# rvp-group/mad-icp

Hardware: NVIDIA H100
Metric: scans/sec (130k-pt scan vs 16-keyframe model) (higher is better)
Workload: dtype f64

## Files before the change

mad_icp_b200/csrc/capi.cu:

```cuda
#include <cooperative_groups.h>
#include <cuda_runtime.h>

#include <algorithm>
#include <cmath>
#include <cstdio>
#include <cstdlib>
#include <cstring>
#include <new>
#include <stdexcept>
#include <string>
#include <vector>

#include "../../include/madicp_b200_debug.h"
#include "ctx.hpp"
#include "device_kernels.cuh"

namespace madicp {

static thread_local std::string g_error;
void set_error(const std::string& msg) { g_error = msg; }

}

using namespace madicp;

ModelView madicp_make_view(const madicp_ctx* c) {
  ModelView v;
  v.recs = c->d_pool_recs;
  v.quad = c->d_quad;
  v.ww = c->d_pool_ww;
  v.K = 0;
  for (int s = 0; s < c->max_keyframes; ++s)
    if (c->slots[s].n_nodes > 0) {
      v.broot[v.K] = int(size_t(s) * c->pool_cap);
      v.qroot[v.K] = int(size_t(s) * c->quad_cap);
      ++v.K;
    }
  for (int i = v.K; i < kMaxSlots; ++i) v.broot[i] = v.qroot[i] = 0;
  return v;
}
static ModelView make_view(const madicp_ctx* c) { return madicp_make_view(c); }

static int blocks_for(int64_t n) { return int((n + kStepBlock - 1) / kStepBlock); }

static int prepare_slot(madicp_ctx* c, int s) {
  const int n = c->slots[s].n_nodes;
  const size_t off = size_t(s) * c->pool_cap;
  k_prepare_slot<<<blocks_for(n), kStepBlock, 0, c->stream>>>(
      c->d_pool_recs + off, n, int(off), c->P.min_ball, c->d_pool_lvl + size_t(s) * (kMaxLevels + 1),
      c->slots[s].n_levels, c->d_pool_child0 + off, c->d_pool_rec_of + off, c->d_quad + size_t(s) * c->quad_cap,
      c->d_pool_ww + off);
  c->launches++;
  CK(cudaGetLastError());
  return MADICP_OK;
}

static int build_slot(madicp_ctx* c, int s, const madtree_rec_t* src, const double* X_dev) {
  const int n = c->slots[s].n_nodes;
  const size_t off = size_t(s) * c->pool_cap;
  const int* lvl = c->d_pool_lvl + size_t(s) * (kMaxLevels + 1);
  const int nl = c->slots[s].n_levels;
  madtree_rec_t* dst = c->d_pool_recs + off;
  k_slot_ingest<<<blocks_for(n), kStepBlock, 0, c->stream>>>(src ? src : dst, dst, n, X_dev, lvl, nl, c->d_pool_child0 + off);
  k_quad_scan<<<1, 1024, 0, c->stream>>>(c->d_pool_child0 + off, n);
  k_quad_place<<<blocks_for(n), kStepBlock, 0, c->stream>>>(dst, n, lvl, nl, c->d_pool_child0 + off, c->d_pool_rec_of + off);
  c->launches += 3;
  CK(cudaGetLastError());
  return prepare_slot(c, s);
}

static int ensure_pool(madicp_ctx* c, size_t need) {
  if (need <= c->pool_cap) return MADICP_OK;
  CK(cudaStreamSynchronize(c->stream));
  size_t cap = size_t(1) << 16;
  while (cap + 40 < need || cap + 40 <= c->pool_cap) cap <<= 1;
  cap += 40;
  if (cap * size_t(c->max_keyframes) > size_t(0x3fffffff)) {
    set_error("keyframe pool would exceed 2^30 nodes");
    return MADICP_ERR_NOMEM;
  }
  madtree_rec_t* recs = nullptr;
  int *child0 = nullptr, *rec_of = nullptr;
  QuadRec* quad = nullptr;
  double* ww = nullptr;
  const size_t total = cap * size_t(c->max_keyframes);
  CK(cudaMalloc(&recs, total * sizeof(madtree_rec_t)));
  CK(cudaMalloc(&child0, total * sizeof(int)));
  CK(cudaMalloc(&rec_of, total * sizeof(int)));
  CK(cudaMalloc(&quad, 2 * total * sizeof(QuadRec)));
  CK(cudaMalloc(&ww, total * sizeof(double)));
  for (int s = 0; s < c->max_keyframes; ++s)
    if (c->slots[s].n_nodes > 0)
      CK(cudaMemcpyAsync(recs + size_t(s) * cap, c->d_pool_recs + size_t(s) * c->pool_cap,
                         size_t(c->slots[s].n_nodes) * sizeof(madtree_rec_t), cudaMemcpyDeviceToDevice, c->stream));
  CK(cudaStreamSynchronize(c->stream));
  cudaFree(c->d_pool_recs);
  cudaFree(c->d_pool_child0);
  cudaFree(c->d_pool_rec_of);
  cudaFree(c->d_quad);
  cudaFree(c->d_pool_ww);
  c->d_pool_ww = ww;
  c->d_pool_recs = recs;
  c->d_pool_child0 = child0;
  c->d_pool_rec_of = rec_of;
  c->d_quad = quad;
  c->quad_cap = 2 * cap;
  c->pool_cap = cap;
  for (int s = 0; s < c->max_keyframes; ++s)
    if (c->slots[s].n_nodes > 0) {
      int rc = build_slot(c, s, nullptr, nullptr);
      if (rc) return rc;
    }
  return MADICP_OK;
}

static int stage_pose(madicp_ctx* c, const double X[12], const double** X_dev) {
  const int r = int(c->xform_seq % madicp_ctx::kXformRing);
  if (c->xform_seq >= madicp_ctx::kXformRing) CK(cudaEventSynchronize(c->xform_done[r]));
  memcpy(c->h_xform + size_t(r) * 12, X, 12 * sizeof(double));
  CK(cudaMemcpyAsync(c->d_xform + size_t(r) * 12, c->h_xform + size_t(r) * 12, 12 * sizeof(double), cudaMemcpyHostToDevice,
                     c->stream));
  CK(cudaEventRecord(c->xform_done[r], c->stream));
  *X_dev = c->d_xform + size_t(r) * 12;
  c->xform_seq++;
  return MADICP_OK;
}

static int slot_rank(const madicp_ctx* c, int slot) {
  int k = 0;
  for (int s = 0; s < slot; ++s) k += (c->slots[s].n_nodes > 0);
  return k;
}

static int ensure_items(madicp_ctx* c, size_t items) {
  if (items <= c->cap_items) return MADICP_OK;
  CK(cudaStreamSynchronize(c->stream));
  if (c->d_hit) cudaFree(c->d_hit);
  if (c->d_ord) cudaFree(c->d_ord);
  c->d_hit = c->d_ord = nullptr;
  c->cap_items = 0;
  CK(cudaMalloc(&c->d_hit, items * sizeof(int)));
  CK(cudaMalloc(&c->d_ord, items * sizeof(int)));
  c->cap_items = items;
  return MADICP_OK;
}

struct GnShape {
  int threads, ctas;
  const void* fn;
  size_t smem;
};
template <int THREADS, int CTAS>
static GnShape gn_shape() {
  return GnShape{THREADS, CTAS, reinterpret_cast<const void*>(k_gn_loop<THREADS, CTAS>), gn_dynamic_smem<THREADS>()};
// ... 88 lines not shown
  c->max_keyframes = max_keyframes;
  c->sm_count = prop.multiProcessorCount;
  c->slots.resize(max_keyframes);
  {
    int lo_pri = 0, hi_pri = 0;
    CK(cudaDeviceGetStreamPriorityRange(&lo_pri, &hi_pri));
    CK(cudaStreamCreateWithPriority(&c->own_stream, cudaStreamNonBlocking, hi_pri));
  }
  c->stream = c->own_stream;
  CK(cudaMalloc(&c->d_state, sizeof(GnState)));
  CK(cudaMemset(c->d_state, 0, sizeof(GnState)));
  CK(cudaMalloc(&c->d_X, sizeof(double) * 64));
  CK(cudaMalloc(&c->d_comm, sizeof(CommBlock)));
  CK(cudaMemset(c->d_comm, 0, sizeof(CommBlock)));
  CK(cudaEventCreateWithFlags(&c->tree_free_ev, cudaEventDisableTiming));
  CK(cudaMalloc(&c->d_pool_lvl, size_t(max_keyframes) * (kMaxLevels + 1) * sizeof(int)));
  CK(cudaMalloc(&c->d_xform, size_t(madicp_ctx::kXformRing) * 12 * sizeof(double)));
  CK(cudaMallocHost(&c->h_xform, size_t(madicp_ctx::kXformRing) * 12 * sizeof(double)));
  CK(cudaMallocHost(&c->h_lvl, size_t(madicp_ctx::kXformRing) * (kMaxLevels + 1) * sizeof(int)));
  for (int i = 0; i < madicp_ctx::kXformRing; ++i) CK(cudaEventCreateWithFlags(&c->xform_done[i], cudaEventDisableTiming));
  CK(cudaMallocHost(&c->h_pinned, sizeof(double) * 64));
  CK(cudaMallocHost(&c->h_state, sizeof(GnState)));
  CK(cudaMallocHost(&c->h_matched, kMatchedCap));
  if (const char* e = getenv("MADICP_NO_MEMO")) c->memo_mode = (atoi(e) == 0) ? 2 : 0;
  int threads = 1024, ctas = 1;
  if (const char* e = getenv("MADICP_GN_SHAPE"))
    if (sscanf(e, "%d,%d", &threads, &ctas) == 2) c->gn_auto = false;
  int rc = configure_gn(c, threads, ctas);
  if (rc) return rc;
  c->cap_partial = size_t(c->sm_count) * 8 * kAcc;
  CK(cudaMalloc(&c->d_partial, c->cap_partial * sizeof(double)));
  CK(cudaMalloc(&c->d_tiles, c->cap_partial * sizeof(LLCell)));
  CK(cudaMemset(c->d_tiles, 0, c->cap_partial * sizeof(LLCell)));
  c->peer_comm[0] = c->d_comm;
  *out = c;
  return MADICP_OK;
  MADICP_CATCH("madicp_create")
}

void madicp_destroy(madicp_ctx_t* c) {
  if (!c) return;
  cudaSetDevice(c->device);
  cudaStreamSynchronize(c->stream);
  for (int r = 0; r < c->world; ++r)
    if (c->world > 1 && r != c->rank && c->peer_comm[r]) cudaIpcCloseMemHandle(c->peer_comm[r]);
  madicp_gpu_build_release(c);
  for (madtree_gpu* t : c->tree_cache) delete t;
  for (void* slab : c->tree_slabs) cudaFree(slab);
  cudaFree(c->d_pool_recs);
  cudaFree(c->d_pool_child0);
  cudaFree(c->d_pool_rec_of);
  cudaFree(c->d_pool_lvl);
  cudaFree(c->d_quad);
  cudaFree(c->d_pool_ww);
  cudaFree(c->d_xform);
  cudaFree(c->d_dbg_cta);
  cudaFree(c->d_moving);
  cudaFree(c->d_mov4);
  cudaFree(c->d_step_matched);
  cudaFree(c->d_hit);
  cudaFree(c->d_ord);
  cudaFree(c->d_cloud_q);
  cudaFree(c->d_cloud_o);
  cudaFree(c->d_partial);
  cudaFree(c->d_tiles);
  cudaFree(c->d_memo_leaf);
  cudaFree(c->d_memo_margin);
  cudaFree(c->d_memo_ckpt);
  cudaFree(c->d_memo_ckpt_up);
  cudaFree(c->d_state);
  cudaFree(c->d_X);
  cudaFree(c->d_comm);
  cudaFree(c->d_dbg);
  cudaFreeHost(c->h_xform);
  cudaFreeHost(c->h_lvl);
  cudaFreeHost(c->h_pinned);
  cudaFreeHost(c->h_state);
  for (int i = 0; i < madicp_ctx::kXformRing; ++i)
    if (c->xform_done[i]) cudaEventDestroy(c->xform_done[i]);
  cudaFreeHost(c->h_matched);
  if (c->tree_free_ev) cudaEventDestroy(c->tree_free_ev);
  cudaStreamDestroy(c->own_stream);
  delete c;
}

int madicp_set_params(madicp_ctx_t* c, double min_ball, double rho_ker, double b_ratio) {
  if (!c || !(min_ball > 0) || rho_ker < 0) {
    set_error("madicp_set_params: bad arguments");
    return MADICP_ERR_INVALID;
  }
  const bool reweigh = (min_ball != c->P.min_ball);
  c->P.min_ball = min_ball;
  c->P.rho_ker_sqrt = sqrt(rho_ker);
  c->P.b_ratio = b_ratio;
  c->mov4_stale = true;
  if (reweigh) {
    CK(cudaSetDevice(c->device));
    for (int s = 0; s < c->max_keyframes; ++s)
      if (c->slots[s].n_nodes > 0) {
        int rc = prepare_slot(c, s);
        if (rc) return rc;
      }
  }
  return MADICP_OK;
}

int madicp_set_stream(madicp_ctx_t* c, void* s) {
  if (!c) return MADICP_ERR_INVALID;
  c->stream = s ? static_cast<cudaStream_t>(s) : c->own_stream;
  return MADICP_OK;
}
void* madicp_get_stream(const madicp_ctx_t* c) { return c ? static_cast<void*>(c->stream) : nullptr; }
int madicp_synchronize(madicp_ctx_t* c) {
  if (!c) return MADICP_ERR_INVALID;
  CK(cudaSetDevice(c->device));
  CK(cudaStreamSynchronize(c->stream));
  return MADICP_OK;
}

static int level_table(const madtree_rec_t* recs, int n_nodes, int n_leaves, std::vector<int>& lvl) {
  lvl.clear();
  lvl.push_back(0);
// ... 441 lines not shown
  CK(cudaMemcpyAsync(c->h_pinned, c->d_X, 12 * sizeof(double), cudaMemcpyDeviceToHost, c->stream));
  CK(cudaStreamSynchronize(c->stream));
  memcpy(X, c->h_pinned, 12 * sizeof(double));
  return MADICP_OK;
}

static int register_enqueue(madicp_ctx* c, int iters, const double X0[12], int clear_from) {
  int rc = check_ready(c, "madicp_register");
  if (rc) return rc;
  if (!X0 || iters < 1 || iters > MADICP_MAX_ITERS) {
    set_error("madicp_register: bad arguments (1 <= iters <= 64 per launch)");
    return MADICP_ERR_INVALID;
  }
  CK(cudaSetDevice(c->device));
  rc = prepare_moving(c);
  if (rc) return rc;
  rc = pick_shape(c, int64_t(madicp_num_keyframes(c)) * c->L);
  if (rc) return rc;
  GnArgs A;
  A.model = make_view(c);
  A.P = c->P;
  A.peers.rank = c->rank;
  A.peers.world = c->world;
  A.peers.epoch_base = c->epoch;
  const int mb = int(c->call_seq & 1u);
  for (int r = 0; r < kMaxPeers; ++r) {
    A.peers.box[r] = (r < c->world) ? &c->peer_comm[r]->box : nullptr;
    A.peer_matched[r] = (r < c->world) ? c->peer_comm[r]->matched[mb] : nullptr;
  }
  A.moving = c->d_mov4;
  A.L = c->L;
  A.iters = iters;
  A.clear_from = clear_from;
  A.matched = c->d_comm->matched[mb];
  size_t map_bytes = 0;
  {
    const size_t per_cta = size_t(madicp_num_keyframes(c)) * (size_t(c->L) / size_t(c->gn_grid) + 8) * 4 + 128;
    auto bucket = [](size_t bytes) {
      const size_t kb[] = {8, 16, 32, 64, 100, 132, 164, 196, 228};
      for (size_t b : kb)
        if (bytes + 1024 <= b * 1024) return b;
      return size_t(1 << 20);
    };
    const size_t ctas = size_t(c->gn_grid / c->sm_count);
    if (per_cta <= kGnMapMaxBytes && c->L < (1 << 26) && bucket((c->gn_smem + per_cta) * ctas) == bucket(c->gn_smem * ctas))
      map_bytes = per_cta;
  }
  A.map_in_smem = map_bytes ? 1 : 0;
  {
    const size_t stride = ((size_t(c->max_keyframes) * (c->cap_moving / size_t(c->gn_grid) + 8)) + 31) & ~size_t(31);
    const size_t need = stride * size_t(c->gn_grid);
    if (need > c->cap_memo) {
      CK(cudaStreamSynchronize(c->stream));
      cudaFree(c->d_memo_leaf);
      cudaFree(c->d_memo_margin);
      cudaFree(c->d_memo_ckpt);
      cudaFree(c->d_memo_ckpt_up);
      c->d_memo_leaf = nullptr;
      c->d_memo_margin = nullptr;
      c->d_memo_ckpt = nullptr;
      c->d_memo_ckpt_up = nullptr;
      c->cap_memo = 0;
      const size_t cap = need + need / 4;
      CK(cudaMalloc(&c->d_memo_leaf, cap * sizeof(int)));
      CK(cudaMalloc(&c->d_memo_margin, cap * sizeof(float)));
      CK(cudaMalloc(&c->d_memo_ckpt, cap * sizeof(unsigned)));
      CK(cudaMalloc(&c->d_memo_ckpt_up, cap * sizeof(float)));
      c->cap_memo = cap;
    }
    A.memo_leaf = c->d_memo_leaf;
    A.memo_margin = c->d_memo_margin;
    A.memo_ckpt = c->d_memo_ckpt;
    A.memo_ckpt_up = c->d_memo_ckpt_up;
    A.item_stride = int(stride);
    A.memo_mode = c->memo_mode;
    A.walk_buf = mb;
  }
  A.st = c->d_state;
  A.dbg = c->d_dbg;
  A.dbg_cta = c->d_dbg ? c->d_dbg_cta : nullptr;
  c->epoch += uint32_t(iters);
  A.pose_epoch = c->pose_epoch;
  c->pose_epoch += uint32_t(iters);
  memcpy(A.X0, X0, 12 * sizeof(double));
  A.tiles = c->d_tiles;
  A.zero_next = c->d_comm->matched[mb ^ 1];
  A.zero_bytes = int((std::min(kMatchedCap, c->cap_moving) + 15) & ~size_t(15));
  void* args[] = {&A};
  CK(cudaLaunchCooperativeKernel(c->gn_kernel, dim3(c->gn_grid), dim3(c->gn_threads), args, c->gn_smem + map_bytes, c->stream));
  c->launches++;
  c->last_iters = iters;
  c->call_seq++;
  return MADICP_OK;
}

int madicp_register_async(madicp_ctx_t* c, int iters, const double X0[12]) {
  return register_enqueue(c, iters, X0, iters - 1);
}
int madicp_register_partial_async(madicp_ctx_t* c, int iters, const double X0[12]) {
  return register_enqueue(c, iters, X0, 0);
}

int madicp_register_fetch_weight(madicp_ctx_t* c, double X[12], double H[36], double b[6], uint8_t* matched, int* n_matched,
                                 double* weight) {
  if (!c || c->last_iters < 1) {
    set_error("madicp_register_fetch: nothing was enqueued");
    return MADICP_ERR_STATE;
  }
  CK(cudaSetDevice(c->device));
  CK(cudaMemcpyAsync(c->h_state, c->d_state, offsetof(GnState, X_trace), cudaMemcpyDeviceToHost, c->stream));
  if (matched)
    CK(cudaMemcpyAsync(c->h_matched, c->d_comm->matched[(c->call_seq - 1u) & 1u], size_t(c->L), cudaMemcpyDeviceToHost,
                       c->stream));
  CK(cudaStreamSynchronize(c->stream));
  if (c->h_state->error) {
    set_error("madicp_register: a peer GPU never delivered its H/b tile (rank down, or no matching registration enqueued there)");
    CK(cudaMemsetAsync(&c->d_state->error, 0, sizeof(int), c->stream));
    return MADICP_ERR_COMM;
  }
  if (X) memcpy(X, c->h_state->X_out, 12 * sizeof(double));
  if (H) memcpy(H, c->h_state->H, 36 * sizeof(double));
  if (b) memcpy(b, c->h_state->b, 6 * sizeof(double));
  if (matched) memcpy(matched, c->h_matched, size_t(c->L));
  if (n_matched) *n_matched = c->h_state->n_matched;
  if (weight) *weight = c->h_state->weight;
  return MADICP_OK;
// ... 256 lines not shown
```

mad_icp_b200/csrc/ctx.hpp:

```cpp
#pragma once
#include <cuda_runtime.h>

#include <atomic>
#include <mutex>
#include <new>
#include <stdexcept>
#include <string>
#include <vector>

#include "kernels.cuh"

namespace madicp {
void set_error(const std::string& msg);

constexpr int kMaxLevels = 4096;
struct Slot {
  int n_nodes = 0, n_leaves = 0, n_levels = 0;
};
constexpr size_t kMatchedCap = size_t(1) << 20;

struct CommBlock {
  Mailbox box;
  unsigned char matched[2][kMatchedCap];
};
}

struct madicp_ctx;

struct madtree_gpu {
  madicp_ctx* ctx = nullptr;
  madtree_rec_t* recs = nullptr;
  int* lvl = nullptr;
  int* leaf_of = nullptr;
  size_t cap_nodes = 0;
  void* block = nullptr;
  int n_nodes = 0, n_leaves = 0, n_levels = 0;
  std::vector<int> h_lvl;
  double* full = nullptr;
  int64_t n_points = 0;
  uint64_t build_seq = 0;
};

struct madicp_ctx {
  int device = 0;
  int max_keyframes = 0;
  cudaStream_t own_stream = nullptr, stream = nullptr;
  int sm_count = 0;
  std::vector<madicp::Slot> slots;
  size_t pool_cap = 0;
  madtree_rec_t* d_pool_recs = nullptr;
  int* d_pool_child0 = nullptr;
  int* d_pool_rec_of = nullptr;
  int* d_pool_lvl = nullptr;
  size_t quad_cap = 0;
  madicp::QuadRec* d_quad = nullptr;
  double* d_pool_ww = nullptr;
  static constexpr int kXformRing = 64;
  double* d_xform = nullptr;
  double* h_xform = nullptr;
  int* h_lvl = nullptr;
  cudaEvent_t xform_done[kXformRing] = {};
  uint32_t xform_seq = 0;
  std::vector<madtree_gpu*> tree_cache;
  std::vector<void*> tree_slabs;
  cudaEvent_t tree_free_ev = nullptr;
  std::mutex tree_mu;
  void* build_state = nullptr;
  long long* d_dbg_cta = nullptr;
  madicp::IcpParams P{0.2, 0.31622776601683794, 0.02};
  double* d_moving = nullptr;
  madicp::Moving4* d_mov4 = nullptr;
  bool mov4_stale = true;
  unsigned char* d_step_matched = nullptr;
  int L = 0;
  size_t cap_moving = 0;
  uint32_t call_seq = 0;
  int* d_hit = nullptr;
  int* d_ord = nullptr;
  size_t cap_items = 0;
  double* d_cloud_q = nullptr;
  int* d_cloud_o = nullptr;
  size_t cap_cloud = 0;
  double* d_partial = nullptr;
  madicp::LLCell* d_tiles = nullptr;
  size_t cap_partial = 0;
  int* d_memo_leaf = nullptr;
  float* d_memo_margin = nullptr;
  unsigned* d_memo_ckpt = nullptr;
  float* d_memo_ckpt_up = nullptr;
  size_t cap_memo = 0;
  int memo_mode = 2;
  madicp::GnState* d_state = nullptr;
  double* d_X = nullptr;
  madicp::CommBlock* d_comm = nullptr;
  double* h_pinned = nullptr;
  madicp::GnState* h_state = nullptr;
  unsigned char* h_matched = nullptr;
  int gn_grid = 0;
  bool gn_auto = true;
  int gn_threads = 1024;
  const void* gn_kernel = nullptr;
  size_t gn_smem = 0;
  static constexpr int kNumAutoShapes = 6;
  static constexpr int kAutoShapes[kNumAutoShapes] = {768, 1024, 896, 704, 640, 512};
  double pass_cost[kNumAutoShapes] = {5570.0, 8260.0, 7480.0, 5650.0, 5325.0, 4650.0};
  bool calibrated = false;
  int last_iters = 0;
  long long* d_dbg = nullptr;
  std::atomic<int64_t> launches{0};
  int rank = 0, world = 1;
  madicp::CommBlock* peer_comm[madicp::kMaxPeers] = {};
  uint32_t epoch = 0;
  uint32_t pose_epoch = 1;
};

#define CK(call)                                                                                   \
  do {                                                                                             \
    cudaError_t e_ = (call);                                                                       \
    if (e_ != cudaSuccess) {                                                                       \
      madicp::set_error(std::string(#call) + ": " + cudaGetErrorString(e_));                       \
      return MADICP_ERR_CUDA;                                                                      \
    }                                                                                              \
  } while (0)

#define MADICP_TRY try {
#define MADICP_CATCH(who)                                          \
  }                                                                \
  catch (const std::bad_alloc&) {                                  \
    madicp::set_error(std::string(who) + ": out of host memory");  \
    return MADICP_ERR_NOMEM;                                       \
  }                                                                \
  catch (const std::exception& e_) {                               \
    madicp::set_error(std::string(who) + ": " + e_.what());        \
    return MADICP_ERR_INVALID;                                     \
  }

int madicp_tree_alloc(madicp_ctx* c, size_t cap_nodes, madtree_gpu** out);
void madicp_gpu_build_release(madicp_ctx* c);
```

mad_icp_b200/csrc/device_kernels.cuh:

```cuda
#pragma once
#include "kernels.cuh"

namespace madicp {


__device__ __forceinline__ int depth_of(const int* __restrict__ lvl, int n_levels, int i) {
  int lo = 0, hi = n_levels;
  while (hi - lo > 1) {
    const int mid = (lo + hi) >> 1;
    if (__ldg(lvl + mid) <= i) lo = mid; else hi = mid;
  }
  return lo;
}

__global__ void __launch_bounds__(kStepBlock)
k_slot_ingest(const madtree_rec_t* src, madtree_rec_t* dst, int n, const double* __restrict__ Xp,
              const int* __restrict__ lvl, int n_levels, int* __restrict__ flag) {
  const int i = blockIdx.x * kStepBlock + threadIdx.x;
  if (i >= n) return;
  Rec r = load_rec_plain(src + i);
  const int npts = src[i].num_points;
  int f = 0;
  if (r.link >= 0 && (depth_of(lvl, n_levels, i) & 1) == 0)
    f = (src[r.link].link >= 0 || src[r.link + 1].link >= 0) ? 1 : 0;
// ... 50 lines not shown
      s_warp[lane] = w;
    }
    __syncthreads();
    int run = s_carry + (warp ? s_warp[warp - 1] : 0) + (incl - mine);
#pragma unroll
    for (int j = 0; j < 4; ++j) {
      if (i0 + j < n) flag_to_child0[i0 + j] = 1 + 4 * run;
      run += f[j];
    }
    __syncthreads();
    if (threadIdx.x == 1023) s_carry = run;
    __syncthreads();
  }
}

__global__ void __launch_bounds__(kStepBlock)
k_quad_place(const madtree_rec_t* __restrict__ recs, int n, const int* __restrict__ lvl, int n_levels,
             const int* __restrict__ child0, int* __restrict__ rec_of) {
  const int i = blockIdx.x * kStepBlock + threadIdx.x;
  if (i >= n) return;
  if (i == 0) rec_of[0] = 0;
  const int l0 = recs[i].link;
  if (l0 < 0 || (depth_of(lvl, n_levels, i) & 1)) return;
  const int c0 = child0[i];
#pragma unroll
  for (int s0 = 0; s0 < 2; ++s0) {
    const int l1 = recs[l0 + s0].link;
    if (l1 < 0) continue;
    rec_of[l1] = c0 + 2 * s0;
    rec_of[l1 + 1] = c0 + 2 * s0 + 1;
  }
}

__device__ __forceinline__ FastRec make_shadow(const Rec& r, int pool_index, double min_ball) {
  FastRec f;
  if (r.link >= 0) {
    f.dx = __double2float_rn(r.dx);
    f.dy = __double2float_rn(r.dy);
    f.dz = __double2float_rn(r.dz);
    f.c = __double2float_rn(dot3(r.mx, r.my, r.mz, r.dx, r.dy, r.dz));
  } else {
    const double w = 1.0 - r.bbox0 / min_ball;
    const double ww = w * w;
    f.dx = __int_as_float(pool_index);
    f.dy = __uint_as_float(kLeafMarker);
    f.dz = __int_as_float(__double2loint(ww));
    f.c = __int_as_float(__double2hiint(ww));
  }
  return f;
}

__global__ void __launch_bounds__(kStepBlock)
k_prepare_slot(const madtree_rec_t* __restrict__ recs, int n, int off, double min_ball, const int* __restrict__ lvl,
               int n_levels, const int* __restrict__ child0, const int* __restrict__ rec_of, QuadRec* __restrict__ quad,
               double* __restrict__ ww_out) {
  const int i = blockIdx.x * kStepBlock + threadIdx.x;
  if (i >= n) return;
  const Rec r = load_rec(recs + i);
  if (r.link < 0) {
    const double w = 1.0 - r.bbox0 / min_ball;
    ww_out[i] = w * w;
  }
  if (depth_of(lvl, n_levels, i) & 1) return;
  QuadRec q;
  q.p0 = make_shadow(r, off + i, min_ball);
  q.p1 = q.p0;
  q.p2 = q.p0;
  q.bfs0 = off + i;
  q.child0 = 0;
  q.pad[0] = q.pad[1] = 0;
  if (r.link >= 0) {
    q.p1 = make_shadow(load_rec(recs + r.link), off + r.link, min_ball);
    q.p2 = make_shadow(load_rec(recs + r.link + 1), off + r.link + 1, min_ball);
    q.child0 = child0[i];
  }
  quad[rec_of[i]] = q;
}

__global__ void __launch_bounds__(kStepBlock)
k_leaf_table(const madtree_rec_t* __restrict__ recs, int n, int* __restrict__ leaf_of) {
  const int i = blockIdx.x * kStepBlock + threadIdx.x;
  if (i >= n) return;
  const int link = recs[i].link;
  if (link < 0) leaf_of[-1 - link] = i;
}

__global__ void __launch_bounds__(kStepBlock)
k_prepare_moving(double* __restrict__ means, int L, const __grid_constant__ IcpParams P, Moving4* __restrict__ out,
                 const madtree_rec_t* __restrict__ recs, const int* __restrict__ leaf_of) {
  const int q = blockIdx.x * kStepBlock + threadIdx.x;
  if (q >= L) return;
  Moving4 m;
  if (recs) {
    const madtree_rec_t* r = recs + leaf_of[q];
    means[3 * q] = r->mean[0];
    means[3 * q + 1] = r->mean[1];
    means[3 * q + 2] = r->mean[2];
  }
  m.px = means[3 * q];
  m.py = means[3 * q + 1];
  m.pz = means[3 * q + 2];
  m.ball = P.min_ball + P.b_ratio * norm3(m.px, m.py, m.pz);
  out[q] = m;
}


__global__ void __launch_bounds__(kStepBlock)
k_search(const __grid_constant__ ModelView model, const Moving4* __restrict__ moving, int L,
         const double* __restrict__ Xp, int* __restrict__ hit, int* __restrict__ ordinals) {
  double X[12];
#pragma unroll
  for (int i = 0; i < 12; ++i) X[i] = Xp[i];
  const unsigned total = unsigned(model.K) * unsigned(L);
  for (unsigned w = blockIdx.x * kStepBlock + threadIdx.x; w < total; w += gridDim.x * kStepBlock) {
    const unsigned k = w / unsigned(L), q = w - k * unsigned(L);
// ... 82 lines not shown

template <int THREADS>
__device__ __forceinline__ void peer_allreduce(const PeerView& pv, uint32_t epoch, double* s_tot,
                                               double (*s_peer)[kAcc], int* error) {
  const int slot = int(epoch & 1u);
  for (int idx = threadIdx.x; idx < pv.world * kAcc; idx += THREADS) {
    const int r = idx / kAcc, i = idx - r * kAcc;
    const double v = s_tot[i];
    const uint32_t lo = uint32_t(__double2loint(v)), hi = uint32_t(__double2hiint(v));
    LLCell* dst = &pv.box[r]->cell[slot][pv.rank][i];
    asm volatile("st.volatile.global.v4.u32 [%0], {%1,%2,%3,%4};" ::"l"(dst), "r"(lo), "r"(epoch), "r"(hi), "r"(epoch)
                 : "memory");
  }
  for (int idx = threadIdx.x; idx < pv.world * kAcc; idx += THREADS) {
    const int r = idx / kAcc, i = idx - r * kAcc;
    const LLCell* src = &pv.box[pv.rank]->cell[slot][r][i];
    uint32_t lo, f0, hi, f1, spins = 0;
    do {
      asm volatile("ld.volatile.global.v4.u32 {%0,%1,%2,%3}, [%4];" : "=r"(lo), "=r"(f0), "=r"(hi), "=r"(f1) : "l"(src)
                   : "memory");
      if (++spins == (1u << 26)) {
        *error = 1;
        break;
      }
    } while (f0 != epoch || f1 != epoch);
    s_peer[r][i] = __hiloint2double(int(hi), int(lo));
  }
  __syncthreads();
  if (threadIdx.x < kAcc) {
    double s = s_peer[0][threadIdx.x];
    for (int r = 1; r < pv.world; ++r) s += s_peer[r][threadIdx.x];
    s_tot[threadIdx.x] = s;
  }
  __syncthreads();
}

struct GnArgs {
  ModelView model;
  IcpParams P;
  PeerView peers;
  const Moving4* moving;
  int L;
  int iters;
  int clear_from;
  unsigned char* matched;
  unsigned char* peer_matched[kMaxPeers];
  LLCell* tiles;
  double X0[12];
  unsigned char* zero_next;
  int zero_bytes;
  GnState* st;
  int map_in_smem;
  uint32_t pose_epoch;
  int* memo_leaf;
  float* memo_margin;
  unsigned* memo_ckpt;
  float* memo_ckpt_up;
  int item_stride;
  int walk_buf;
  int memo_mode;
  long long* dbg;
  long long* dbg_cta;
};
#ifndef MADICP_CKPT_TAU_SCALE
#define MADICP_CKPT_TAU_SCALE 1.0
#endif
__device__ __forceinline__ float ckpt_tau(int it, double moved, double ball) {
  return __double2float_ru(MADICP_CKPT_TAU_SCALE * (it == 0 ? ball : moved));
}

__device__ __forceinline__ long long global_ns() {
  long long t;
  asm volatile("mov.u64 %0, %%globaltimer;" : "=l"(t));
  return t;
}

template <int THREADS, int CTAS>
__global__ void __launch_bounds__(THREADS, CTAS)
k_gn_loop(const __grid_constant__ GnArgs A) {
  constexpr int WARPS = THREADS / 32;
  extern __shared__ __align__(16) double s_dyn[];
  double* s_stage_all = s_dyn;
  double(*s_red)[64] = reinterpret_cast<double(*)[64]>(s_dyn);
  double(*s_peer)[kAcc] = reinterpret_cast<double(*)[kAcc]>(s_dyn + WARPS * 64);
  static_assert(WARPS * 64 + kMaxPeers * kAcc <= WARPS * kStageTile, "scratch must fit in the staging tiles");
  __shared__ double s_tot[kAcc];
  __shared__ double s_b[6];
  __shared__ double s_X[12], s_Xp[12];
  __shared__ int s_qn, s_rn;
  __shared__ int s_count[WARPS];
  GnState* st = A.st;
  const unsigned L = unsigned(A.L);
  const unsigned total = unsigned(A.model.K) * L;
  const bool multi = A.peers.world > 1;
  const unsigned lane = threadIdx.x & 31;
  const unsigned warp = threadIdx.x >> 5;
  double* stage = s_stage_all + warp * kStageTile;
  constexpr unsigned kPieces = 4;
  unsigned p_lo[kPieces], p_n[kPieces];
  unsigned n_b = 0;
#pragma unroll
  const unsigned G = gridDim.x;
  const unsigned light = (G >= 8u) ? 3u : 0u;
  const uint64_t W8 = 8ull * G - light;
  for (unsigned p = 0; p < kPieces; ++p) {
    const unsigned s = (p & 1u) ? (G - 1u - blockIdx.x) : blockIdx.x;
    auto cum8 = [&](unsigned pos) -> uint64_t {
      if (p & 1u) return (pos >= G) ? W8 : 8ull * pos;
      return pos ? 8ull * pos - light : 0ull;
    };
    const uint64_t p0 = (uint64_t(L) * p) / kPieces, p1 = (uint64_t(L) * (p + 1)) / kPieces;
    const unsigned lo = unsigned(p0 + ((p1 - p0) * cum8(s)) / W8);
    const unsigned hi = unsigned(p0 + ((p1 - p0) * cum8(s + 1u)) / W8);
    p_lo[p] = lo;
    p_n[p] = hi - lo;
    n_b += p_n[p];
  }
  const unsigned t_total = unsigned(A.model.K) * n_b;
  (void) total;
  auto item_of = [&](unsigned t0, unsigned& k, unsigned& q) {
    k = t0 / n_b;
    q = t0 - k * n_b + lane;
    while (q >= n_b) {
      q -= n_b;
      ++k;
    }
    const unsigned j = q;
    q = p_lo[kPieces - 1] + (j - (n_b - p_n[kPieces - 1]));
    unsigned acc = 0;
#pragma unroll
    for (unsigned p = 0; p + 1 < kPieces; ++p) {
      if (j >= acc && j < acc + p_n[p]) q = p_lo[p] + (j - acc);
      acc += p_n[p];
    }
  };
  unsigned* s_map = A.map_in_smem ? reinterpret_cast<unsigned*>(s_dyn + WARPS * kStageTile) : nullptr;
  if (s_map) {
    for (unsigned t0 = warp * 32; t0 < t_total; t0 += THREADS) {
      unsigned k, q;
      item_of(t0, k, q);
      s_map[t0 + lane] = (k << 26) | q;
    }
    __syncwarp();
  }

  for (int i = (blockIdx.x * THREADS + threadIdx.x) * 16; i < A.zero_bytes; i += gridDim.x * THREADS * 16)
    *reinterpret_cast<uint4*>(A.zero_next + i) = make_uint4(0, 0, 0, 0);
  if (blockIdx.x == 0 && threadIdx.x < MADICP_MAX_ITERS) {
    st->walked[A.walk_buf ^ 1][threadIdx.x] = 0;
    st->walk_recs[A.walk_buf ^ 1][threadIdx.x] = 0;
  }
  int* const memo_leaf = A.memo_leaf + size_t(blockIdx.x) * A.item_stride;
  float* const memo_margin = A.memo_margin + size_t(blockIdx.x) * A.item_stride;
  unsigned* const memo_ckpt = A.memo_ckpt + size_t(blockIdx.x) * A.item_stride;
  float* const memo_ckpt_up = A.memo_ckpt_up + size_t(blockIdx.x) * A.item_stride;
  auto item_at = [&](unsigned t0, unsigned& k, unsigned& q) {
    if (s_map) {
      const unsigned pk = s_map[t0 + lane];
      k = pk >> 26;
      q = pk & 0x3ffffffu;
    } else {
      item_of(t0, k, q);
    }
  };

  for (int it = 0; it < A.iters; ++it) {
    if (threadIdx.x < 12) {
      double x;
      if (it == 0) {
        x = A.X0[threadIdx.x];
      } else {
        const uint32_t ep = A.pose_epoch + uint32_t(it);
        uint32_t lo, hi, f0, f1;
        do {
          ll_load(&st->X_ll[threadIdx.x], lo, f0, hi, f1);
        } while (f0 != ep || f1 != ep);
        x = __hiloint2double(int(hi), int(lo));
      }
      s_Xp[threadIdx.x] = s_X[threadIdx.x];
      s_X[threadIdx.x] = x;
      if (it == 0 && blockIdx.x == 0) st->X_trace[threadIdx.x] = x;
    }
    if (threadIdx.x == 32) s_qn = 0;
    if (threadIdx.x == 33) s_rn = 0;
    __syncthreads();
    const bool last_round = (it == A.iters - 1);
    double c0 = 0.0, c1 = 0.0;
    long long t_begin = 0;
    if (A.dbg && threadIdx.x == 0) t_begin = clock64();
    const size_t dbg_plane = size_t(MADICP_MAX_ITERS) * gridDim.x, dbg_at = size_t(it) * gridDim.x + blockIdx.x;
    if (A.dbg_cta && threadIdx.x == 0) A.dbg_cta[dbg_plane + dbg_at] = global_ns();

    int n_walked = 0, n_recs = 0;
    for (unsigned t0 = warp * 32; t0 < t_total; t0 += THREADS) {
      unsigned k, q;
      item_at(t0, k, q);
      double v[kStage];
#pragma unroll
      for (int i = 0; i < kStage; ++i) v[i] = 0.0;
      const unsigned t = t0 + lane;
      if (t < t_total) {
        const Moving4 m = load_moving(A.moving + q);
        double mx, my, mz;
        iso_apply(s_X, m.px, m.py, m.pz, mx, my, mz);
        int leaf = -1;
        Rec f;
        double ww = 0.0;
        unsigned start = 0;
        float prefix = __int_as_float(0x7f800000);
        double moved = 0.0;
        if (it > 0 && A.memo_mode) {
          const float have = memo_margin[t];
          const int last = memo_leaf[t];
          unsigned ck = 0;
          float ck_up = 0.0f;
          if (A.memo_mode == 2) {
            ck = memo_ckpt[t];
            ck_up = memo_ckpt_up[t];
          }
          f = load_rec(A.model.recs + last);
          ww = __ldg(A.model.ww + last);
          double bx, by, bz;
          iso_apply(s_Xp, m.px, m.py, m.pz, bx, by, bz);
          const double dx = mx - bx, dy = my - by, dz = mz - bz;
          moved = 1.0001 * sqrt(dx * dx + dy * dy + dz * dz) + 1e-9 + 1e-12 * (fabs(mx) + fabs(my) + fabs(mz));
          const double left = double(have) - moved;
          if (left > 0.0) {
            memo_margin[t] = __double2float_rd(left);
            leaf = last;
          } else if (ck != 0) {
            const double ck_left = __dsub_rd(__dadd_rd(double(have), double(ck_up)), moved);
            if (ck_left > 0.0) {
              start = ck;
              prefix = __double2float_rd(ck_left);
            }
          }
        }
        if (leaf < 0) {
          double ww_walk;
          const float tau = ckpt_tau(it, moved, m.ball);
          float margin = prefix, ck_margin = 0.0f;
          unsigned ckpt = start;
          leaf = A.memo_mode ? descend_t<true>(A.model, int(k), mx, my, mz, ww_walk, margin, ckpt, ck_margin, tau, n_recs)
                             : descend_t<false>(A.model, int(k), mx, my, mz, ww_walk, margin, ckpt, ck_margin, tau, n_recs);
          if (A.memo_mode) {
            memo_leaf[t] = leaf;
            memo_margin[t] = margin;
          }
          if (A.memo_mode == 2) {
            memo_ckpt[t] = ckpt;
            memo_ckpt_up[t] = __fsub_rd(ck_margin, margin);
          }
          ++n_walked;
          ww = __ldg(A.model.ww + leaf);
          f = load_rec(A.model.recs + leaf);
        }
        if (linearize_one(s_X, A.P.rho_ker_sqrt, m, mx, my, mz, f, ww, v) && it >= A.clear_from) {
          if (multi) {
            for (int r = 0; r < A.peers.world; ++r) A.peer_matched[r][q] = 1;
          } else {
            A.matched[q] = 1;
          }
        }
      }
      warp_accumulate(stage, v, c0, c1);
    }
    n_walked = __reduce_add_sync(0xffffffffu, n_walked);
    n_recs = __reduce_add_sync(0xffffffffu, n_recs);
    if (lane == 0 && n_walked) {
      atomicAdd(&s_qn, n_walked);
      atomicAdd(&s_rn, n_recs);
    }
    if (A.dbg && threadIdx.x == 0 && blockIdx.x == 0) A.dbg[it * 8 + 0] = clock64() - t_begin;
    if (A.dbg_cta) {
      __syncthreads();
      if (threadIdx.x == 0) {
        A.dbg_cta[dbg_at] = clock64() - t_begin;
        A.dbg_cta[2 * dbg_plane + dbg_at] = global_ns();
      }
      if (threadIdx.x == 0 && blockIdx.x == 0) A.dbg[it * 8 + 5] = s_qn;
    }
    __syncthreads();
    if (threadIdx.x == 0 && s_qn) {
      atomicAdd(&st->walked[A.walk_buf][it], s_qn);
      atomicAdd(&st->walk_recs[A.walk_buf][it], (unsigned long long) s_rn);
    }
    const uint32_t ep_round = A.pose_epoch + uint32_t(it);
    block_reduce_publish<WARPS>(c0, c1, s_red, A.tiles + size_t(blockIdx.x) * kAcc, ep_round,
                                 it >= A.clear_from, multi);
    if (A.dbg_cta && threadIdx.x == 0) A.dbg_cta[3 * dbg_plane + dbg_at] = global_ns();
    if (blockIdx.x == 0) {
      long long t0 = 0, t1 = 0, t2 = 0;
      if (A.dbg && threadIdx.x == 0) t0 = clock64();
      fold_tiles<THREADS>(A.tiles, gridDim.x, ep_round, s_red, s_tot,
                          (A.dbg_cta && gridDim.x >= 16) ? A.dbg_cta + 4 * dbg_plane + size_t(it) * gridDim.x : nullptr);
      if (A.dbg && threadIdx.x == 0) {
        t1 = clock64();
        A.dbg[it * 8 + 1] = t1 - t_begin;
        A.dbg[it * 8 + 2] = t1 - t0;
        A.dbg[it * 8 + 6] = global_ns();
      }
      if (multi) {
        if (last_round) __threadfence_system();
        peer_allreduce<THREADS>(A.peers, A.peers.epoch_base + uint32_t(it) + 1u, s_tot, s_peer, &st->error);
        if (last_round) __threadfence_system();
      }
      if (last_round) {
        __threadfence();
// ... 55 lines not shown
```

mad_icp_b200/csrc/kernels.cuh:

```cuda
#pragma once
#include <cuda_runtime.h>
#include <stdint.h>

#include "../../include/madicp_b200.h"
#include "arith.h"
#include "solve6.h"

namespace madicp {

constexpr int kMaxSlots = 64;
constexpr int kStepBlock = 256;
constexpr int kAcc = 48;
constexpr int kStage = 13;
constexpr int kStageItems = 16;
constexpr int kStagePitch = 20;
constexpr int kStageTile = kStage * kStagePitch;
constexpr int kMaxPeers = 16;
constexpr int kMailboxSlots = 2;

struct __align__(16) FastRec {
  float dx, dy, dz, c;
};
static_assert(sizeof(FastRec) == 16, "FastRec must be one 128-bit load");

constexpr float kBoundC = 1.0e-6f;

struct __align__(32) QuadRec {
  FastRec p0, p1, p2;
  int bfs0;
  int child0;
  int pad[2];
};
static_assert(sizeof(QuadRec) == 64, "QuadRec must be four 128-bit loads");

struct ModelView {
  const madtree_rec_t* recs;
  const QuadRec* quad;
  const double* ww;
  int broot[kMaxSlots];
  int qroot[kMaxSlots];
  int K;
};
constexpr unsigned kLeafMarker = 0x7fc0beefu;

struct IcpParams {
  double min_ball, rho_ker_sqrt, b_ratio;
};

struct __align__(32) Moving4 {
  double px, py, pz, ball;
};

struct __align__(16) LLCell {
  uint32_t lo, flag_lo, hi, flag_hi;
};

__device__ __forceinline__ void ll_store(LLCell* p, double v, uint32_t epoch) {
  asm volatile("st.volatile.global.v4.u32 [%0], {%1,%2,%3,%4};" ::"l"(p), "r"(uint32_t(__double2loint(v))), "r"(epoch),
               "r"(uint32_t(__double2hiint(v))), "r"(epoch) : "memory");
}
__device__ __forceinline__ void ll_load(const LLCell* p, uint32_t& lo, uint32_t& f0, uint32_t& hi, uint32_t& f1) {
  asm volatile("ld.volatile.global.v4.u32 {%0,%1,%2,%3}, [%4];" : "=r"(lo), "=r"(f0), "=r"(hi), "=r"(f1) : "l"(p) : "memory");
}

struct GnState {
  int ticket;
  int clear_from;
  int n_matched;
  int error;
  double X_in[12];
  double X_out[12];
  double H[36];
  double b[6];
  double weight;
  double X_trace[(MADICP_MAX_ITERS + 1) * 12];
  int walked[2][MADICP_MAX_ITERS];
  unsigned long long walk_recs[2][MADICP_MAX_ITERS];
  LLCell X_ll[12];
};

struct Mailbox {
  LLCell cell[kMailboxSlots][kMaxPeers][kAcc];
};

struct PeerView {
  Mailbox* box[kMaxPeers];
  int rank, world;
  uint32_t epoch_base;
};

struct Rec {
// ... 359 lines not shown
```

Baseline: 4993.

## Cache matched leaf geometry and weight per item in a planar double2 memo

```diff
diff --git a/mad_icp_b200/csrc/capi.cu b/mad_icp_b200/csrc/capi.cu
--- a/mad_icp_b200/csrc/capi.cu
+++ b/mad_icp_b200/csrc/capi.cu
@@ -28,7 +28,6 @@
   ModelView v;
   v.recs = c->d_pool_recs;
   v.quad = c->d_quad;
-  v.ww = c->d_pool_ww;
   v.K = 0;
   for (int s = 0; s < c->max_keyframes; ++s)
     if (c->slots[s].n_nodes > 0) {
@@ -48,8 +47,7 @@
   const size_t off = size_t(s) * c->pool_cap;
   k_prepare_slot<<<blocks_for(n), kStepBlock, 0, c->stream>>>(
       c->d_pool_recs + off, n, int(off), c->P.min_ball, c->d_pool_lvl + size_t(s) * (kMaxLevels + 1),
-      c->slots[s].n_levels, c->d_pool_child0 + off, c->d_pool_rec_of + off, c->d_quad + size_t(s) * c->quad_cap,
-      c->d_pool_ww + off);
+      c->slots[s].n_levels, c->d_pool_child0 + off, c->d_pool_rec_of + off, c->d_quad + size_t(s) * c->quad_cap);
   c->launches++;
   CK(cudaGetLastError());
   return MADICP_OK;
@@ -82,13 +80,11 @@
   madtree_rec_t* recs = nullptr;
   int *child0 = nullptr, *rec_of = nullptr;
   QuadRec* quad = nullptr;
-  double* ww = nullptr;
   const size_t total = cap * size_t(c->max_keyframes);
   CK(cudaMalloc(&recs, total * sizeof(madtree_rec_t)));
   CK(cudaMalloc(&child0, total * sizeof(int)));
   CK(cudaMalloc(&rec_of, total * sizeof(int)));
   CK(cudaMalloc(&quad, 2 * total * sizeof(QuadRec)));
-  CK(cudaMalloc(&ww, total * sizeof(double)));
   for (int s = 0; s < c->max_keyframes; ++s)
     if (c->slots[s].n_nodes > 0)
       CK(cudaMemcpyAsync(recs + size_t(s) * cap, c->d_pool_recs + size_t(s) * c->pool_cap,
@@ -98,8 +94,6 @@
   cudaFree(c->d_pool_child0);
   cudaFree(c->d_pool_rec_of);
   cudaFree(c->d_quad);
-  cudaFree(c->d_pool_ww);
-  c->d_pool_ww = ww;
   c->d_pool_recs = recs;
   c->d_pool_child0 = child0;
   c->d_pool_rec_of = rec_of;
@@ -294,7 +288,6 @@
   cudaFree(c->d_pool_rec_of);
   cudaFree(c->d_pool_lvl);
   cudaFree(c->d_quad);
-  cudaFree(c->d_pool_ww);
   cudaFree(c->d_xform);
   cudaFree(c->d_dbg_cta);
   cudaFree(c->d_moving);
@@ -306,10 +299,9 @@
   cudaFree(c->d_cloud_o);
   cudaFree(c->d_partial);
   cudaFree(c->d_tiles);
+  cudaFree(c->d_memo_margin);
   cudaFree(c->d_memo_leaf);
-  cudaFree(c->d_memo_margin);
-  cudaFree(c->d_memo_ckpt);
-  cudaFree(c->d_memo_ckpt_up);
+  cudaFree(c->d_pair);
   cudaFree(c->d_state);
   cudaFree(c->d_X);
   cudaFree(c->d_comm);
@@ -857,26 +849,23 @@
     const size_t need = stride * size_t(c->gn_grid);
     if (need > c->cap_memo) {
       CK(cudaStreamSynchronize(c->stream));
+      cudaFree(c->d_memo_margin);
       cudaFree(c->d_memo_leaf);
-      cudaFree(c->d_memo_margin);
-      cudaFree(c->d_memo_ckpt);
-      cudaFree(c->d_memo_ckpt_up);
+      cudaFree(c->d_pair);
+      c->d_memo_margin = nullptr;
       c->d_memo_leaf = nullptr;
-      c->d_memo_margin = nullptr;
-      c->d_memo_ckpt = nullptr;
-      c->d_memo_ckpt_up = nullptr;
+      c->d_pair = nullptr;
       c->cap_memo = 0;
       const size_t cap = need + need / 4;
+      CK(cudaMalloc(&c->d_memo_margin, cap * sizeof(float)));
       CK(cudaMalloc(&c->d_memo_leaf, cap * sizeof(int)));
-      CK(cudaMalloc(&c->d_memo_margin, cap * sizeof(float)));
-      CK(cudaMalloc(&c->d_memo_ckpt, cap * sizeof(unsigned)));
-      CK(cudaMalloc(&c->d_memo_ckpt_up, cap * sizeof(float)));
+      CK(cudaMalloc(&c->d_pair, 4 * cap * sizeof(double2)));
       c->cap_memo = cap;
     }
+    A.memo_margin = c->d_memo_margin;
     A.memo_leaf = c->d_memo_leaf;
-    A.memo_margin = c->d_memo_margin;
-    A.memo_ckpt = c->d_memo_ckpt;
-    A.memo_ckpt_up = c->d_memo_ckpt_up;
+    A.pair = c->d_pair;
+    A.pair_plane = c->cap_memo;
     A.item_stride = int(stride);
     A.memo_mode = c->memo_mode;
     A.walk_buf = mb;
diff --git a/mad_icp_b200/csrc/ctx.hpp b/mad_icp_b200/csrc/ctx.hpp
--- a/mad_icp_b200/csrc/ctx.hpp
+++ b/mad_icp_b200/csrc/ctx.hpp
@@ -54,7 +54,6 @@
   int* d_pool_lvl = nullptr;
   size_t quad_cap = 0;
   madicp::QuadRec* d_quad = nullptr;
-  double* d_pool_ww = nullptr;
   static constexpr int kXformRing = 64;
   double* d_xform = nullptr;
   double* h_xform = nullptr;
@@ -84,10 +83,9 @@
   double* d_partial = nullptr;
   madicp::LLCell* d_tiles = nullptr;
   size_t cap_partial = 0;
+  float* d_memo_margin = nullptr;
   int* d_memo_leaf = nullptr;
-  float* d_memo_margin = nullptr;
-  unsigned* d_memo_ckpt = nullptr;
-  float* d_memo_ckpt_up = nullptr;
+  double2* d_pair = nullptr;
   size_t cap_memo = 0;
   int memo_mode = 2;
   madicp::GnState* d_state = nullptr;
diff --git a/mad_icp_b200/csrc/device_kernels.cuh b/mad_icp_b200/csrc/device_kernels.cuh
--- a/mad_icp_b200/csrc/device_kernels.cuh
+++ b/mad_icp_b200/csrc/device_kernels.cuh
@@ -126,15 +126,10 @@
 
 __global__ void __launch_bounds__(kStepBlock)
 k_prepare_slot(const madtree_rec_t* __restrict__ recs, int n, int off, double min_ball, const int* __restrict__ lvl,
-               int n_levels, const int* __restrict__ child0, const int* __restrict__ rec_of, QuadRec* __restrict__ quad,
-               double* __restrict__ ww_out) {
+               int n_levels, const int* __restrict__ child0, const int* __restrict__ rec_of, QuadRec* __restrict__ quad) {
   const int i = blockIdx.x * kStepBlock + threadIdx.x;
   if (i >= n) return;
   const Rec r = load_rec(recs + i);
-  if (r.link < 0) {
-    const double w = 1.0 - r.bbox0 / min_ball;
-    ww_out[i] = w * w;
-  }
   if (depth_of(lvl, n_levels, i) & 1) return;
   QuadRec q;
   q.p0 = make_shadow(r, off + i, min_ball);
@@ -323,10 +318,10 @@
   GnState* st;
   int map_in_smem;
   uint32_t pose_epoch;
+  float* memo_margin;
   int* memo_leaf;
-  float* memo_margin;
-  unsigned* memo_ckpt;
-  float* memo_ckpt_up;
+  double2* pair;
+  size_t pair_plane;
   int item_stride;
   int walk_buf;
   int memo_mode;
@@ -338,6 +333,13 @@
 #endif
 __device__ __forceinline__ float ckpt_tau(int it, double moved, double ball) {
   return __double2float_ru(MADICP_CKPT_TAU_SCALE * (it == 0 ? ball : moved));
+}
+
+__device__ __forceinline__ void ld_f64x2(const double2* p, double& a, double& b) {
+  asm volatile("ld.global.v2.f64 {%0,%1}, [%2];" : "=d"(a), "=d"(b) : "l"(p));
+}
+__device__ __forceinline__ void st_cs_f64x2(double2* p, double a, double b) {
+  asm volatile("st.global.cs.v2.f64 [%0], {%1,%2};" ::"l"(p), "d"(a), "d"(b) : "memory");
 }
 
 __device__ __forceinline__ long long global_ns() {
@@ -421,10 +423,9 @@
     st->walked[A.walk_buf ^ 1][threadIdx.x] = 0;
     st->walk_recs[A.walk_buf ^ 1][threadIdx.x] = 0;
   }
+  float* const memo_margin = A.memo_margin + size_t(blockIdx.x) * A.item_stride;
   int* const memo_leaf = A.memo_leaf + size_t(blockIdx.x) * A.item_stride;
-  float* const memo_margin = A.memo_margin + size_t(blockIdx.x) * A.item_stride;
-  unsigned* const memo_ckpt = A.memo_ckpt + size_t(blockIdx.x) * A.item_stride;
-  float* const memo_ckpt_up = A.memo_ckpt_up + size_t(blockIdx.x) * A.item_stride;
+  double2* const pair = A.pair + size_t(blockIdx.x) * A.item_stride;
   auto item_at = [&](unsigned t0, unsigned& k, unsigned& q) {
     if (s_map) {
       const unsigned pk = s_map[t0 + lane];
@@ -474,7 +475,7 @@
         const Moving4 m = load_moving(A.moving + q);
         double mx, my, mz;
         iso_apply(s_X, m.px, m.py, m.pz, mx, my, mz);
-        int leaf = -1;
+        bool kept = false;
         Rec f;
         double ww = 0.0;
         unsigned start = 0;
@@ -483,14 +484,17 @@
         if (it > 0 && A.memo_mode) {
           const float have = memo_margin[t];
           const int last = memo_leaf[t];
-          unsigned ck = 0;
-          float ck_up = 0.0f;
-          if (A.memo_mode == 2) {
-            ck = memo_ckpt[t];
-            ck_up = memo_ckpt_up[t];
+          double ckw;
+          ld_f64x2(pair + t + 3 * A.pair_plane, ww, ckw);
+          if (last < 0) {
+            ld_f64x2(pair + t, f.mx, f.my);
+            ld_f64x2(pair + t + A.pair_plane, f.mz, f.dx);
+            ld_f64x2(pair + t + 2 * A.pair_plane, f.dy, f.dz);
+          } else {
+            f = load_rec(A.model.recs + last);
           }
-          f = load_rec(A.model.recs + last);
-          ww = __ldg(A.model.ww + last);
+          const unsigned ck = unsigned(__double2loint(ckw));
+          const float ck_up = __int_as_float(__double2hiint(ckw));
           double bx, by, bz;
           iso_apply(s_Xp, m.px, m.py, m.pz, bx, by, bz);
           const double dx = mx - bx, dy = my - by, dz = mz - bz;
@@ -498,7 +502,13 @@
           const double left = double(have) - moved;
           if (left > 0.0) {
             memo_margin[t] = __double2float_rd(left);
-            leaf = last;
+            kept = true;
+            if (last >= 0 && !last_round) {
+              st_cs_f64x2(pair + t, f.mx, f.my);
+              st_cs_f64x2(pair + t + A.pair_plane, f.mz, f.dx);
+              st_cs_f64x2(pair + t + 2 * A.pair_plane, f.dy, f.dz);
+              memo_leaf[t] = -1;
+            }
           } else if (ck != 0) {
             const double ck_left = __dsub_rd(__dadd_rd(double(have), double(ck_up)), moved);
             if (ck_left > 0.0) {
@@ -507,24 +517,21 @@
             }
           }
         }
-        if (leaf < 0) {
-          double ww_walk;
+        if (!kept) {
           const float tau = ckpt_tau(it, moved, m.ball);
           float margin = prefix, ck_margin = 0.0f;
           unsigned ckpt = start;
-          leaf = A.memo_mode ? descend_t<true>(A.model, int(k), mx, my, mz, ww_walk, margin, ckpt, ck_margin, tau, n_recs)
-                             : descend_t<false>(A.model, int(k), mx, my, mz, ww_walk, margin, ckpt, ck_margin, tau, n_recs);
-          if (A.memo_mode) {
+          const int leaf = A.memo_mode
+                               ? descend_t<true>(A.model, int(k), mx, my, mz, ww, margin, ckpt, ck_margin, tau, n_recs)
+                               : descend_t<false>(A.model, int(k), mx, my, mz, ww, margin, ckpt, ck_margin, tau, n_recs);
+          ++n_walked;
+          f = load_rec(A.model.recs + leaf);
+          if (A.memo_mode && !last_round) {
+            memo_margin[t] = margin;
             memo_leaf[t] = leaf;
-            memo_margin[t] = margin;
+            if (A.memo_mode == 1) ckpt = 0;
+            st_cs_f64x2(pair + t + 3 * A.pair_plane, ww, __hiloint2double(__float_as_int(__fsub_rd(ck_margin, margin)), int(ckpt)));
           }
-          if (A.memo_mode == 2) {
-            memo_ckpt[t] = ckpt;
-            memo_ckpt_up[t] = __fsub_rd(ck_margin, margin);
-          }
-          ++n_walked;
-          ww = __ldg(A.model.ww + leaf);
-          f = load_rec(A.model.recs + leaf);
         }
         if (linearize_one(s_X, A.P.rho_ker_sqrt, m, mx, my, mz, f, ww, v) && it >= A.clear_from) {
           if (multi) {
diff --git a/mad_icp_b200/csrc/kernels.cuh b/mad_icp_b200/csrc/kernels.cuh
--- a/mad_icp_b200/csrc/kernels.cuh
+++ b/mad_icp_b200/csrc/kernels.cuh
@@ -36,7 +36,6 @@
 struct ModelView {
   const madtree_rec_t* recs;
   const QuadRec* quad;
-  const double* ww;
   int broot[kMaxSlots];
   int qroot[kMaxSlots];
   int K;
```

Result: faster. 5056, median of 6 (+1.3%).
